# sidfeels/cosmos-predict2.5

Hardware: AMD Instinct MI355X
Metric: frames/sec, Predict2.5-2B Image2World 720p×121f, 35 UniPC steps, CP=1/8 (higher is better)
Workload: dtype bf16

## Files before the change

cosmos-predict2.5_amd/cosmos_predict2/_native.py:

```python

from __future__ import annotations

import ctypes
import os
from typing import Optional, Tuple

import torch

_DEFAULT_LIB_PATH = os.path.join(os.path.dirname(os.path.abspath(__file__)), "_lib", "libcp25.so")
_LIB_PATH = _DEFAULT_LIB_PATH
_lib: Optional[ctypes.CDLL] = None

c_int64_p = ctypes.POINTER(ctypes.c_int64)


class UniPCParams(ctypes.Structure):

    _fields_ = [
        ("sigma", ctypes.c_float),
        ("use_corr", ctypes.c_int),
        ("order_c", ctypes.c_int),
        ("c_a", ctypes.c_float),
        ("c_b", ctypes.c_float),
        ("c_c", ctypes.c_float),
# ... 21 lines not shown


DT_BF16, DT_F32, DT_F8E4M3, DT_U8 = 1, 2, 3, 4
_DTYPES = {torch.bfloat16: DT_BF16, torch.float32: DT_F32, torch.float8_e4m3fn: DT_F8E4M3, torch.uint8: DT_U8}

_P = ctypes.c_void_p
_I64 = ctypes.c_int64
_I = ctypes.c_int
_F = ctypes.c_float
_D = ctypes.c_double
_T =ctypes.POINTER(CP25Tensor)

SIGNATURES = {
    "cp25_attn_fwd": [_P, _P, _P, _P, _I, _I, _I, _I, _I, c_int64_p, c_int64_p, c_int64_p, c_int64_p, _F, _P],
    "cp25_attn_fwd_split": [_P, _P, _P, _P, _I, _I, _I, _I, _I, c_int64_p, c_int64_p, c_int64_p, c_int64_p, _F, _I,
                            _P, ctypes.c_size_t, _P],
    "cp25_attn_fwd_bounded": [_P, _P, _P, _P, _I, _I, _I, _I, _I, c_int64_p, c_int64_p, c_int64_p, c_int64_p, _F, _F,
                              _F, _I, _P, ctypes.c_size_t, _P],
    "cp25_attn_fwd_prescaled_kslots": [_P, _P, _P, _P, _I, _I, _I, _I, _I, c_int64_p, c_int64_p, c_int64_p, c_int64_p,
                                       _F, _F, _P, _I, _I, _P, ctypes.c_size_t, _P],
    "cp25_attn_fwd_prescaled": [_P, _P, _P, _P, _I, _I, _I, _I, _I, c_int64_p, c_int64_p, c_int64_p, c_int64_p, _F,
                                _F, _I, _P, ctypes.c_size_t, _P],
    "cp25_attn_fwd_prescaled_fp8qk": [_P, _P, _P, _P, _I, _I, _I, _I, _I, c_int64_p, c_int64_p, c_int64_p, c_int64_p, _F,
                                _F, _I, _P, ctypes.c_size_t, _P],
    "cp25_cast_fp8_e4m3": [_P, _I64, _P, _I64, _I64, _I64, _F, _P],
    "cp25_attn_fwd_prescaled_fp8": [_P, _P, _P, _P, _P, _I, _I, _I, _I, _I, c_int64_p, c_int64_p, c_int64_p, _F, _F, _I,
                                    _P, ctypes.c_size_t, _P],
    "cp25_v_fp8t_bytes": [_I, _I, _I],
    "cp25_cast_v_fp8t": [_P, c_int64_p, _I, _I, _I, _I, _P, _P, _P],
    "cp25_attn_fwd_prescaled_qnorm": [_P, _P, _P, _P, _I, _I, _I, _I, _I, c_int64_p, c_int64_p, c_int64_p, c_int64_p, _F,
                                      _F, _P, _I, _P, _P, _P, _F, _F, _I, _P, ctypes.c_size_t, _P],
    "cp25_attn_workspace_bytes": [_I, _I, _I, _I],
    "cp25_attn_tail_workspace_bytes": [_I, _I, _I, _I],
    "cp25_attn_kernel": [_I, _F, _F, _F, _I, _I],
    "cp25_attn_plan": [_I, _I, _I, _I, _I],
    "cp25_attn_na3d": [_P, _P, _P, _P, _I, _I, _I, _I, _I, _I, c_int64_p, c_int64_p, c_int64_p, c_int64_p, _P, _P, _I, _I,
                       ctypes.POINTER(ctypes.c_int), ctypes.POINTER(ctypes.c_int), _F, _I, _P],
    "cp25_ln_mod": [_P, _I64, _I64, _P, _P, _P, _P, _I64, _I64, _P, _P, _I64, _I, _I, _I64, _I64, _F, _P],
    "cp25_ln_mod_fp8": [_P, _I64, _I64, _P, _P, _P, _P, _I64, _I64, _P, _P, _P, _I64, _I, _I, _I64, _I64, _F, _P],
    "cp25_ln_mod_cam": [_P, _I64, _I64, _P, _P, _P, _P, _I64, _I64, _P, _I64, _I64, _P, _P, _I64, _I, _I, _I64, _I64, _F,
                        _P],
    "cp25_ln_mod_cam_fp8": [_P, _I64, _I64, _P, _P, _P, _P, _I64, _I64, _P, _I64, _I64, _P, _P, _P, _I64, _I, _I, _I64,
                            _I64, _F, _P],
    "cp25_plucker_tokens": [_P, _P, _P, _I, _I, _I, _P],
    "cp25_final_ln_mod": [_P, _P, _P, _I64, _I64, _P, _P, _I64, _I64, _P, _I64, _I, _I, _I64, _I64, _F, _P],
    "cp25_layer_norm": [_P, _I64, _P, _P, _P, _I64, _I64, _I, _F, _P],
    "cp25_head_rmsnorm_rope": [_P, _I64, _I64, _I, _I, _I, _P, _P, _P, _P, _I64, _F, _P],
    "cp25_head_rmsnorm_rope_scaled": [_P, _I64, _I64, _I, _I, _I, _P, _P, _P, _P, _I64, _F, _F, _P],
    "cp25_head_rmsnorm_rope_nmax": [_P, _I64, _I64, _I, _I, _I, _P, _P, _P, _P, _I64, _F, _F, _P, _P],
    "cp25_copy_rows": [_P, _I64, _P, _I64, _I64, _I64, _P],
    "cp25_gelu": [_P, _I64, _P],
    "cp25_gemm_epi": [_P, _I64, _P, _I64, _P, _I64, _I, _I, _I, _I, _P],
    "cp25_gemm_f32": [_P, _I64, _I64, _P, _I64, _I64, _P, _I64, _I64, _P, _I64, _I64, _I, _I, _I, _I, _I, _P, _I64,
                      _P],
    "cp25_gemm_f32_workspace_floats": [_I, _I, _I, _I],
    "cp25_gemm_hnorm": [_P, _I64, _P, _I64, _P, _I64, _I, _I, _I, _P, _F, _F, _P],
    "cp25_gemm_qkv": [_P, _I64, _P, _I64, _P, _I64, _I, _I, _I, _I, _I, _P, _P, _P, _I, _F, _P],
    "cp25_gemm_res": [_P, _I64, _P, _I64, _P, _I64, _I, _I, _I, _P, _I64, _I64, _P, _I64, _I64, _I, _I64, _I64, _P],
    "cp25_gemm_fp8": [_P, _I64, _P, _P, _I64, _P, _P, _I64, _I, _I, _I, _P],
    "cp25_gemm_fp8_res": [_P, _I64, _P, _P, _I64, _P, _P, _I64, _I, _I, _I, _P, _I64, _I64, _P, _I64, _I64, _I, _I64,
                          _I64, _P],
    "cp25_quant_fp8_rows": [_P, _P, _P, _I64, _I64, _P],
    "cp25_gelu_quant_fp8": [_P, _P, _P, _I64, _I64, _P],
    "cp25_patchify": [_P, _P, _P, _P, _P, _I64, _I64, _I64, _P],
    "cp25_patchify_ld": [_P, _P, _P, _P, _P, _I64, _I64, _I64, _I64, _P],
    "cp25_cfg_velocity": [_P, _I, _P, _P, _P, _F, _I, _P, _I64, _I64, _I64, _P],
# ... 17 lines not shown
    "cp25_gemm_epi_t": [_T, _T, _T, _I, _P],
    "cp25_conv3d_t": [_T, _I, _T, _T, _T, _I, _I, _I, _I, _I, _I, _P],
    "cp25_resize_crop_u8": [_P, c_int64_p, _I, _I, _I, _I, _P, c_int64_p, _P, _P, _P, _I, _P, _P, _P, _I, _I, _I, _I,
                            _I, _I, _I, _P],
    "cp25_u8_to_clip": [_P, c_int64_p, _I, _I, _I, _I, _P, _P],
    "cp25_clip_to_u8": [_P, c_int64_p, _I, _I, _I, _I, _P, c_int64_p, _P],
    "cp25_lora_merge": [_P, _I64, _P, _P, _I64, _I64, _I, _F, _P],
}


def library_path() -> str:
    return _LIB_PATH


def load_library() -> ctypes.CDLL:
    global _lib
    if _lib is not None:
        return _lib
    if not os.path.exists(_LIB_PATH):
        raise RuntimeError(
            f"libcp25.so not found at {_LIB_PATH}: build it with `make -C cosmos-predict2.5_amd/csrc` "
            "(or __graft_entry__.build()). There is no non-native fallback."
        )
    lib = ctypes.CDLL(_LIB_PATH)
    lab = os.path.abspath(_LIB_PATH) != os.path.abspath(_DEFAULT_LIB_PATH)
    for name, argtypes in SIGNATURES.items():
        fn = getattr(lib, name, None)
        if fn is None:
            if argtypes is None or lab:
                continue
            raise RuntimeError(f"libcp25.so does not export {name}")
        if argtypes is not None:
            fn.argtypes = argtypes
        fn.restype = {"cp25_attn_workspace_bytes": ctypes.c_size_t, "cp25_attn_tail_workspace_bytes": ctypes.c_size_t, "cp25_v_fp8t_bytes": ctypes.c_int64,
                      "cp25_gemm_f32_workspace_floats": ctypes.c_int64,
                      "cp25_attn_kernel": ctypes.c_char_p,
                      "cp25_vae_attn_workspace_bytes": ctypes.c_int64}.get(name, ctypes.c_int)
    _lib = lib
    return lib


_ERRORS = {-22: "invalid shape/stride/pointer", -95: "unsupported dtype/size", -5: "kernel launch failed"}


def _check(name: str, rc: int) -> None:
    if rc != 0:
        msg = f"{name} failed with code {rc} ({_ERRORS.get(rc, 'unknown')})"
        if rc == -5:
            raise RuntimeError(msg)
        raise ValueError(msg)


def _ptr(t: Optional[torch.Tensor]) -> Optional[int]:
    if t is None:
        return None
    if not t.is_cuda:
        raise RuntimeError("cp25 kernels need device (HBM) tensors; got a CPU tensor")
    return t.data_ptr()


def _stream(device: torch.device) -> int:
    return torch.cuda.current_stream(device).cuda_stream


def tensor_desc(t: Optional[torch.Tensor]) -> Optional[CP25Tensor]:
    if t is None:
        return None
# ... 55 lines not shown


def attn_plan(B: int, H: int, Lq: int, Lk: int, D: int = 128) -> int:
    n = load_library().cp25_attn_plan(B, H, Lq, Lk, D)
    _check("cp25_attn_plan", min(n, 0))
    return n


def attn_fwd(q: torch.Tensor, k: torch.Tensor, v: torch.Tensor, out: Optional[torch.Tensor] = None,
             softmax_scale: Optional[float] = None, n_split: Optional[int] = None,
             norm_bounds: Optional[Tuple[float, float]] = None, prescaled: bool = False,
             fp8_qk: Optional[Tuple[torch.Tensor, torch.Tensor]] = None,
             fp8_v: Optional[Tuple[torch.Tensor, torch.Tensor]] = None,
             k_norm_slots: Optional[torch.Tensor] = None, q_norm: Optional[dict] = None) -> torch.Tensor:
    lib = load_library()
    if q.dtype != torch.bfloat16 or k.dtype != torch.bfloat16 or v.dtype != torch.bfloat16:
        raise ValueError("attn_fwd expects bf16 q/k/v (attention() recasts to bf16 first)")
    B, Lq, H, D = q.shape
    Bk, Lk, Hk, Dk = k.shape
    if (Bk, Hk, Dk) != (B, H, D) or tuple(v.shape) != tuple(k.shape):
        raise ValueError(f"shape mismatch q{tuple(q.shape)} k{tuple(k.shape)} v{tuple(v.shape)}")
    for t in (q, k, v):
        if t.stride(3) != 1:
            raise ValueError("head dim must be contiguous")
    if out is None:
        out = torch.empty((B, Lq, H, D), dtype=torch.bfloat16, device=q.device)
    scale = float(D) ** -0.5 if softmax_scale is None else float(softmax_scale)
    planned = n_split is None and not _ATTN_SPLIT
    if n_split is None:
        n_split = min(_ATTN_SPLIT, (Lk + 63) // 64) if _ATTN_SPLIT else attn_plan(B, H, Lq, Lk, D)
    ws_bytes = lib.cp25_attn_workspace_bytes(B, H, Lq, n_split)
    if planned and n_split == 1 and fp8_qk is None and k_norm_slots is None:
        ws_bytes = lib.cp25_attn_tail_workspace_bytes(B, H, Lq, Lk)
    ws = torch.empty(((ws_bytes + 15) // 16 * 4,), dtype=torch.float32, device=q.device) if ws_bytes else None
    qb, kb = (0.0, 0.0) if norm_bounds is None else (float(norm_bounds[0]), float(norm_bounds[1]))
    if not (qb >= 0.0 and kb >= 0.0):
        raise ValueError(f"norm_bounds must be >= 0, got {norm_bounds}")
    strides = [_i64x3((t.stride(0), t.stride(1), t.stride(2))) for t in (q, k, v, out)]
    if prescaled:
        if fp8_qk is not None:
            if q_norm is not None:
                raise ValueError("q_norm: the fp8 forms read e4m3 copies of the normalised q")
            if qb * kb > 60.0 or qb <= 0.0 or kb <= 0.0:
                raise ValueError(f"fp8 Q K^T needs norm bounds with product <= 60, got {norm_bounds}")
            q8, k8 = fp8_qk
            if q8.dtype != torch.uint8 or k8.dtype != torch.uint8 or q8.shape != q.shape or k8.shape != k.shape:
                raise ValueError("fp8_qk: uint8 (e4m3 bit pattern) views shaped like q and k expected")
            if q8.stride(3) != 1 or k8.stride(3) != 1:
                raise ValueError("fp8_qk: head dim must be contiguous")
            strides[0] = _i64x3((q8.stride(0), q8.stride(1), q8.stride(2)))
            strides[1] = _i64x3((k8.stride(0), k8.stride(1), k8.stride(2)))
            if fp8_v is not None:
                if 1.13 * qb * kb > 30.0:
                    raise ValueError(f"fp8 P.V needs 1.13 x the norm-bound product <= 30, got {norm_bounds}")
                v8t, amax = fp8_v
                if v8t.dtype != torch.uint8 or v8t.numel() != lib.cp25_v_fp8t_bytes(B, H, Lk) or \
                        amax.dtype != torch.float32 or amax.numel() < B * H:
                    raise ValueError("fp8_v: (v8t uint8 of cp25_v_fp8t_bytes, v_amax float32 [B*H]) expected")
                rc = lib.cp25_attn_fwd_prescaled_fp8(_ptr(q8), _ptr(k8), _ptr(v8t), _ptr(amax), _ptr(out), B, H, Lq, Lk,
                                                     D, strides[0], strides[1], strides[3], qb, kb, int(n_split),
                                                     _ptr(ws), ws_bytes, _stream(q.device))
                _check("cp25_attn_fwd_prescaled_fp8", rc)
                return out
            rc = lib.cp25_attn_fwd_prescaled_fp8qk(_ptr(q8), _ptr(k8), _ptr(v), _ptr(out), B, H, Lq, Lk, D, *strides,
                                                   qb, kb, int(n_split), _ptr(ws), ws_bytes, _stream(q.device))
            _check("cp25_attn_fwd_prescaled_fp8qk", rc)
# ... 803 lines not shown
```

cosmos-predict2.5_amd/csrc/attn_common.h:

```cpp
#pragma once
#include "cp25_common.h"

#include <algorithm>
#include <type_traits>

namespace cp25attn {

constexpr int kD = 128;
constexpr int kWaves = 8;
constexpr int kQRows = 32;
constexpr int kQBlk = kWaves * kQRows;
constexpr int kKBlk = 64;
constexpr int kThreads = kWaves * 64;
constexpr float kTop = 96.f;
constexpr float kMaxBound = 98.f;
constexpr float kPDrop = 60.f;
constexpr float kGateFixed = 110.f;
constexpr float kTopF8 = 60.f;
constexpr float kLazy = 24.f;

typedef __attribute__((address_space(3))) const char* lds_char_ptr;

typedef float f32x2 __attribute__((ext_vector_type(2)));
typedef __bf16 bf16x2v __attribute__((ext_vector_type(2)));
// ... 42 lines not shown
  x = fmaxf(__uint_as_float(r[0]), __uint_as_float(r[1]));
  auto s = __builtin_amdgcn_permlane32_swap(__float_as_uint(x), __float_as_uint(x), false, false);
  return fmaxf(__uint_as_float(s[0]), __uint_as_float(s[1]));
}

struct AttnArgs {
  const unsigned short* q; const unsigned short* k; const unsigned short* v; unsigned short* o;
  int64_t q_sb, q_sl, q_sh;
  int64_t k_sb, k_sl, k_sh;
  int64_t v_sb, v_sl, v_sh;
  int64_t o_sb, o_sl, o_sh;
  int B, H, Lq, Lk;
  int nqb;
  int nsplit;
  int tps;
  int ntk_v;
  const float* v_amax;
  float s_init;
  float* o_part;
  float* lse_part;
  float scale_log2;
  float kbound;
  const float* kslots;
  int n_kslots;
  const unsigned short* qn_w;
  const float* qn_cos;
  const float* qn_sin;
  float qn_eps, qn_scale;
  int qn_row0;
#ifdef CP25_ATTN_PROBE
  unsigned long long* probe;
  int probe_t0, probe_wg;
#endif
};

constexpr int kKStride16 = 288;
constexpr int kVStride16 = 288;
constexpr int kKBuf16 = kKBlk * kKStride16;
constexpr int kVBuf16 = kKBlk * kVStride16;
constexpr int kLds16 = 2 * kKBuf16 + 2 * kVBuf16;

typedef void (*AttnKernel)(AttnArgs);
AttnKernel wq_kernel(int rows, int mode, bool tail);
constexpr int kWqThreads = 256;

}
```

cosmos-predict2.5_amd/csrc/attn_fwd.hip:

```cpp
#include "attn_common.h"

namespace {
using namespace cp25attn;

constexpr int kAheadDefault = 2;

constexpr bool kQCopyStagger = true;
constexpr int kOStr = 264;
constexpr int kQSlot = kQRows * kOStr;
constexpr int kLdsP = kLds16 + kWaves * kQSlot;

template <int kKind, bool kPre, int kMode, bool kPersist = false, int kGate = 0, int kTail = 0>
__global__ void __launch_bounds__(kThreads, 2) attn_fwd_m16(AttnArgs a) {
  __shared__ __attribute__((aligned(16))) char smem[kPersist ? kLdsP : kLds16];
  constexpr int KB1 = kKBuf16, VB0 = 2 * kKBuf16;
  static_assert(kMode >= 0 && kMode <= 2 && (kMode != 1 || kPre), "kMode: 0 fixed, 1 zero shift, 2 online");
  static_assert(!kPersist || (kKind == 1 && kMode != 0), "persistent form: cross-attention, zero shift or online");
  constexpr bool online = kMode == 2;
  constexpr bool kInit = kPre && kMode != 1;
  constexpr int kAhead = !kPersist ? 3 : kAheadDefault;

  const int tile = xcd_remap(blockIdx.x, gridDim.x);
  int blk0 = 0, blk_end = 0;
  if constexpr (kPersist) {
// ... 9 lines not shown
  const int Lk = min(a.Lk - key0, a.tps * kKBlk);
  const int ntk = (Lk + kKBlk - 1) / kKBlk;

  const int tid = threadIdx.x;
  const int lane = tid & 63;
  const int wave = tid >> 6;
  const int c16 = lane & 15;
  const int g = lane >> 4;
  const bool group_b = __builtin_amdgcn_readfirstlane(tid) >= kThreads / 2;
  const int wave_u = __builtin_amdgcn_readfirstlane(tid >> 6);
#ifdef CP25_ATTN_PROBE
  __shared__ unsigned long long probe_lds[kWaves * 32 * 4];
  unsigned long long probe_clk[4] = {0, 0, 0, 0};
  unsigned probe_resc = 0;
  const bool probe_on = !kPersist && kTail == 0 && a.probe != nullptr && (int)blockIdx.x < a.probe_wg;
  int probe_t = -1;
  unsigned long long probe_b2 = 0;
#define ATTN_STAMP(T, K)                                                                                    \
  do {                                                                                                      \
    if (probe_on && (unsigned)((T) - a.probe_t0) < 32u) {                                                   \
      __builtin_amdgcn_sched_barrier(0);                                                                    \
      unsigned long long ts_;                                                                               \
      asm volatile("s_memtime %0\n\ts_waitcnt lgkmcnt(0)" : "=s"(ts_)::"memory");                          \
      probe_lds[(wave_u * 32 + (T) - a.probe_t0) * 4 + (K)] = ts_;                                         \
      __builtin_amdgcn_sched_barrier(0);                                                                    \
    }                                                                                                       \
  } while (0)
#else
#define ATTN_STAMP(T, K) \
  do {                   \
  } while (0)
#endif

  const unsigned short* qp = a.q + b * a.q_sb + h * a.q_sh;
  const unsigned short* kp = a.k + b * a.k_sb + h * a.k_sh + (int64_t)key0 * a.k_sl;
  const unsigned short* vp = a.v + b * a.v_sb + h * a.v_sh + (int64_t)key0 * a.v_sl;

  const int ntiles = kPersist ? (blk_end - blk0) * ntk : ntk;
  const int copy_tile = kPersist && ntk > 1 ? (kQCopyStagger ? (int)(blockIdx.x % (unsigned)(ntk - 1)) : 0) : 0;

  const int u = tid & (kThreads / 2 - 1);
  const int srow = u >> 4, sch = u & 15;
  const int64_t sl = group_b ? a.k_sl : a.v_sl;
  const char* sbase = group_b ? (const char*)kp : (const char*)vp;
  const int st_off = (int)(srow * sl * 2) + sch * 16, st_step = (int)(16 * sl * 2);
  u32x4 st[4];
  auto load_tile = [&](int t) __attribute__((always_inline)) {
    const char* base;
    int kt;
    if constexpr (kPersist) {
      const int tb = t / ntk;
      kt = t - tb * ntk;
      const int bh_t = (blk0 + tb) / a.nqb;
      const int b_t = bh_t / a.H, h_t = bh_t % a.H;
      base = group_b ? (const char*)(a.k + b_t * a.k_sb + h_t * a.k_sh) : (const char*)(a.v + b_t * a.v_sb + h_t * a.v_sh);
    } else {
      kt = t;
      base = sbase;
    }
    const int rows = (kPersist && t >= ntiles) ? 0 : min(Lk - kt * kKBlk, kKBlk);
    const int nbytes = rows > 0 ? (int)((rows - 1) * sl * 2) + 2 * kD : 0;
    const auto rsrc = __builtin_amdgcn_make_buffer_rsrc((void*)(base + (int64_t)kt * kKBlk * sl * 2), (short)0, nbytes,
                                                        0x00020000);
    int off = st_off;
    if constexpr (kPersist) {
      const int uf = ((wave_u & 3) << 6) + lane_fresh();
// ... 101 lines not shown
#pragma unroll
          for (int q = 0; q < 4; ++q)
            x[s][q] = hn2_norm(x[s][q], rstd2,
                               f32x2{static_cast<float>(wv[s][2 * q]), static_cast<float>(wv[s][2 * q + 1])});
        f32x2 y[4][4];
#pragma unroll
        for (int s = 0; s < 4; ++s)
#pragma unroll
          for (int q = 0; q < 4; ++q) y[s][q] = x[s][q];
        if (rope) {
#pragma unroll
          for (int s = 0; s < 4; ++s)
#pragma unroll
            for (int q = 0; q < 4; ++q) {
              const f32x4 cc = rc[qh][s & 1][q >> 1], sn = rsn[qh][s & 1][q >> 1];
              const int o = 2 * (q & 1);
              y[s][q] = hn2_rope(x[s][q], x[s ^ 2][q], s < 2 ? -1.f : 1.f, f32x2{cc[o], cc[o + 1]},
                                 f32x2{sn[o], sn[o + 1]});
            }
        }
#pragma unroll
        for (int s = 0; s < 4; ++s)
#pragma unroll
          for (int q = 0; q < 4; ++q) {
            const bf16x2v h = __builtin_convertvector(y[s][q] * scale2, bf16x2v);
            qf[qh][s][2 * q] = h.x;
            qf[qh][s][2 * q + 1] = h.y;
          }
      }
    }
  }

  float gate_kbound = a.kbound;
  if constexpr (kGate != 0) {
    static_assert(kPre && !kPersist && ((kGate == 1 && kMode == 0) || (kGate == 2 && kMode == 2)), "gated pair");
    __shared__ float gate_max[kWaves];
    float km = lane < a.n_kslots ? a.kslots[32 * lane] : 0.f;
    float qm = 0.f;
#pragma unroll
    for (int qh = 0; qh < 2; ++qh) {
      float qq = 0.f;
#pragma unroll
      for (int s = 0; s < 4; ++s)
#pragma unroll
        for (int e = 0; e < 8; ++e) {
          const float x = static_cast<float>(qf[qh][s][e]);
          qq = fmaf(x, x, qq);
        }
      qm = fmaxf(qm, sqrtf(group4_sum(qq)));
    }
#pragma unroll
    for (int m = 32; m >= 1; m >>= 1) {
      km = fmaxf(km, __shfl_xor(km, m));
      qm = fmaxf(qm, __shfl_xor(qm, m));
    }
    if (lane == 0) gate_max[wave] = qm;
    __syncthreads();
#pragma unroll
    for (int w = 0; w < kWaves; ++w) qm = fmaxf(qm, gate_max[w]);
    const bool fixed_ok = km > 0.f && qm * km * 1.001f <= kGateFixed;
    gate_kbound = km * 1.001f;
    if (fixed_ok != (kGate == 1)) {
      if constexpr (kDmaK) asm volatile("s_waitcnt vmcnt(0)" ::: "memory");
      return;
    }
  }

// ... 372 lines not shown
#endif
      mfma_phase(PAR, std::true_type{});
      if constexpr (kDmaK) asm volatile("s_waitcnt vmcnt(0)" ::: "memory");
      __syncthreads();
    };
    for (int t = 0; t + 1 < ntiles; t += 2) {
      step(B0{}, t);
      step(B1{}, t + 1);
    }
    if (ntiles & 1) step(B0{}, ntiles - 1);
  }

#ifdef CP25_ATTN_PROBE
  if (probe_on) {
    asm volatile("s_memtime %0\n\ts_memrealtime %1\n\ts_waitcnt lgkmcnt(0)" : "=s"(probe_clk[2]), "=s"(probe_clk[3])::"memory");
    for (int i = lane; i < 128; i += 64)
      a.probe[((size_t)blockIdx.x * kWaves + wave_u) * 128 + i] = probe_lds[wave_u * 128 + i];
    if (lane < 5)
      a.probe[(size_t)a.probe_wg * kWaves * 128 + ((size_t)blockIdx.x * kWaves + wave_u) * 8 + lane] =
          lane == 0 ? probe_clk[0] : lane == 1 ? probe_clk[1] : lane == 2 ? probe_clk[2] : lane == 3 ? probe_clk[3]
                                                                                                    : probe_resc;
  }
#undef ATTN_STAMP
#endif
  if constexpr (kPersist) {
    store_block(blk_end - 1);
    return;
  }
#pragma unroll
  for (int qh = 0; qh < 2; ++qh) {
    const float l_tot = lsum[qh][0];
    const float inv = 1.f / l_tot;
    if (q_row[qh] >= a.Lq) continue;
    if (a.nsplit > 1) {
      const int64_t row = ((int64_t)(split * a.B + b) * a.H + h) * a.Lq + q_row[qh];
      float* op = a.o_part + row * kD + 4 * g;
#pragma unroll
      for (int db = 0; db < 8; ++db) {
        f32x4 w;
#pragma unroll
        for (int e = 0; e < 4; ++e) w[e] = o[db][qh][e] * inv;
        *reinterpret_cast<f32x4*>(op + 16 * db) = w;
      }
      if (g == 0) a.lse_part[row] = m_run[qh] + __log2f(l_tot);
    } else if constexpr (kKind == 1) {
      store_rows16(a.o + b * a.o_sb + h * a.o_sh + (int64_t)q_row[qh] * a.o_sl, qh, inv, g);
    } else {
      unsigned short* op = a.o + b * a.o_sb + h * a.o_sh + (int64_t)q_row[qh] * a.o_sl + 4 * g;
#pragma unroll
      for (int db = 0; db < 8; ++db) {
        u16x4 w;
#pragma unroll
        for (int e = 0; e < 4; ++e) w[e] = f2bf(o[db][qh][e] * inv);
        *reinterpret_cast<u16x4*>(op + 16 * db) = w;
      }
    }
  }
}

constexpr int kVStride = 320;
constexpr int kVBuf = kKBlk * kVStride;
constexpr int kLdsF8 = 2 * kVBuf + 2 * kKBlk * 144;

template <int kKind, int kF8>
__global__ void __launch_bounds__(kThreads, 2) attn_fwd_f8(AttnArgs a) {
  __shared__ __attribute__((aligned(16))) char smem[kLdsF8];
// ... 398 lines not shown
  double best_cost = 1e300;
  for (int s = 1; s <= 8 && s <= ntiles; ++s) {
    const int64_t tps = cdiv(ntiles, s);
    if (cdiv(ntiles, tps) != s) continue;
    double cost = split_cost(nwg, ntiles, s, rows, cus);
    if (s == 1) {
      TailSeg seg[kMaxTailSegs];
      size_t need;
      double saved;
      if (plan_tail(B, H, Lq, Lk, qblk, seg, &need, &saved) > 0) cost -= saved;
    }
    if (cost < best_cost * 0.995) { best_cost = cost; best = s; }
  }
  return best;
}

int m16_mode(float q_norm_bound, float k_norm_bound, float scale_log2, bool prescaled, bool whole_ok = false) {
  const double bb = (double)q_norm_bound * k_norm_bound * (prescaled ? 1.0 : scale_log2);
  if (!(q_norm_bound > 0.f && k_norm_bound > 0.f)) return 2;
  if (whole_ok && bb <= kGateFixed) return 0;
  if (bb > kMaxBound) return 2;
  return prescaled && bb <= kTop ? 1 : 0;
}

bool m16_gated(float q_norm_bound, float k_norm_bound, bool long_keys) {
  return long_keys ? m16_mode(q_norm_bound, k_norm_bound, 1.f, true, true) == 2
                   : m16_mode(q_norm_bound, k_norm_bound, 1.f, true) != 1;
}

int g_xattn_form = 1;

int wq_default_rows(int Lk) { return Lk > 8192 ? 384 : 320; }
int g_self_form = 1;
int wide_rows(bool prescaled, int fp8, bool gated, int Lk, int mode) {
  if (g_self_form == 0 || !prescaled || fp8 != 0 || gated || Lk <= 4096 || mode == 2) return 0;
  const int rows = g_self_form == 1 ? wq_default_rows(Lk) : g_self_form;
  return wq_kernel(rows, mode, false) ? rows : 0;
}

bool use_xattn_persistent(bool short_keys, int n_split, int mode, int64_t ntiles) {
  return g_xattn_form == 1 && short_keys && n_split == 1 && mode != 0 && ntiles >= 2;
}

}

extern "C" int cp25_attn_self_select(int form) {
  if (form != 0 && form != 1 && !wq_kernel(form, 0, false)) return CP25_ERR_INVAL;
  const int prev = g_self_form;
  g_self_form = form;
  return prev;
}

extern "C" int cp25_attn_cross_select(int form) {
  if (form != 0 && form != 1) return CP25_ERR_INVAL;
  const int prev = g_xattn_form;
  g_xattn_form = form;
  return prev;
}

#ifdef CP25_ATTN_PROBE
static unsigned long long* g_probe = nullptr;
static int g_probe_t0 = 0, g_probe_wg = 0;
extern "C" void cp25_attn_probe_set(unsigned long long* probe, int t0, int n_wg) {
  g_probe = probe;
  g_probe_t0 = t0;
  g_probe_wg = n_wg;
}
#endif

static int attn_launch(const void* q, const void* k, const void* v, void* o, int B, int H, int Lq, int Lk, int D,
                       const int64_t* q_strides, const int64_t* k_strides, const int64_t* v_strides,
// ... 5 lines not shown
  if (D != kD) return CP25_ERR_DTYPE;
  if (fp8qk && !prescaled) return CP25_ERR_INVAL;
  if (fp8 == 2 && (!v_amax || ((uintptr_t)v_amax & 3))) return CP25_ERR_INVAL;
  if (fp8qk && !(q_norm_bound > 0.f && k_norm_bound > 0.f && (double)q_norm_bound * k_norm_bound <= (double)kTopF8))
    return CP25_ERR_INVAL;
  if (fp8 == 2 && 1.13 * (double)q_norm_bound * k_norm_bound > 30.0) return CP25_ERR_INVAL;
  if (B <= 0 || H <= 0 || Lq <= 0 || Lk <= 0) return CP25_ERR_INVAL;
  if (!q || !k || !v || !o) return CP25_ERR_INVAL;
  if (!(softmax_scale > 0.f) || !(q_norm_bound >= 0.f) || !(k_norm_bound >= 0.f) || q_norm_bound > 1e18f ||
      k_norm_bound > 1e18f)
    return CP25_ERR_INVAL;
  const int64_t* ss[4] = {q_strides, k_strides, v_strides, o_strides};
  for (int i = 0; i < 4; ++i)
    for (int j = 0; j < 3; ++j)
      if (!(fp8 == 2 && i == 2) && ss[i][j] % (fp8qk && i < 2 ? 16 : 8) != 0) return CP25_ERR_INVAL;
  if ((int64_t)kKBlk * k_strides[1] * (fp8qk ? 1 : 2) >= (1ll << 31) ||
      (fp8 != 2 && (int64_t)kKBlk * v_strides[1] * 2 >= (1ll << 31)))
    return CP25_ERR_INVAL;
  if (k_strides[1] <= 0 || (fp8 != 2 && v_strides[1] <= 0)) return CP25_ERR_INVAL;
  if (((uintptr_t)q | (uintptr_t)k | (uintptr_t)v | (uintptr_t)o) & 15) return CP25_ERR_INVAL;
  const int64_t ntiles = cdiv(Lk, kKBlk);
  if (n_split < 1 || n_split > ntiles) return CP25_ERR_INVAL;
  const int64_t tps = cdiv(ntiles, n_split);
  if (cdiv(ntiles, tps) != n_split) return CP25_ERR_INVAL;
  const int64_t rows = (int64_t)B * H * Lq;
  if (n_split > 1) {
    if (!workspace || ((uintptr_t)workspace & 15) || ws_bytes < cp25_attn_workspace_bytes(B, H, Lq, n_split))
      return CP25_ERR_INVAL;
  }
  const bool xk = Lk <= 4096;
  const float sl2 = prescaled ? 1.f : softmax_scale * 1.4426950408889634f;
  const int mode = m16_mode(q_norm_bound, k_norm_bound, sl2, prescaled, !xk);
  const bool gated = prescaled && kslots && m16_gated(q_norm_bound, k_norm_bound, !xk);
  const int wq_rows = wide_rows(prescaled, fp8, gated, Lk, mode);
  const int qblk = wq_rows ? wq_rows : kQBlk;
  TailSeg tail[kMaxTailSegs];
  int n_tail = 0;
  if (n_split == 1 && fp8 == 0 && !kslots && workspace && !((uintptr_t)workspace & 15)) {
    size_t need = 0;
    n_tail = plan_tail(B, H, Lq, Lk, qblk, tail, &need, nullptr);
    if (ws_bytes < need) n_tail = 0;
  }
  AttnArgs a;
  a.q = (const unsigned short*)q; a.k = (const unsigned short*)k; a.v = (const unsigned short*)v;
  a.o = (unsigned short*)o;
  a.q_sb = q_strides[0]; a.q_sl = q_strides[1]; a.q_sh = q_strides[2];
  a.k_sb = k_strides[0]; a.k_sl = k_strides[1]; a.k_sh = k_strides[2];
  a.v_sb = v_strides[0]; a.v_sl = v_strides[1]; a.v_sh = v_strides[2];
  a.o_sb = o_strides[0]; a.o_sl = o_strides[1]; a.o_sh = o_strides[2];
  a.B = B; a.H = H; a.Lq = Lq; a.Lk = Lk;
  a.nqb = (int)cdiv(Lq, qblk);
  a.nsplit = n_split;
  a.tps = (int)tps;
  a.ntk_v = (int)ntiles;
  a.v_amax = v_amax;
  a.s_init = fp8 == 2 ? -std::max(0.f, 1.13f * q_norm_bound * k_norm_bound - 15.f) : 0.f;
  a.o_part = n_split > 1 ? (float*)workspace : nullptr;
  a.lse_part = n_split > 1 ? (float*)workspace + (size_t)n_split * rows * kD : nullptr;
  a.scale_log2 = sl2;
  a.kbound = q_norm_bound > 0.f ? k_norm_bound : 0.f;
  a.kslots = kslots;
  a.n_kslots = n_kslots;
  a.qn_w = qn ? qn->qn_w : nullptr;
  a.qn_cos = qn ? qn->qn_cos : nullptr;
  a.qn_sin = qn ? qn->qn_sin : nullptr;
  a.qn_eps = qn ? qn->qn_eps : 0.f;
  a.qn_scale = qn ? qn->qn_scale : 1.f;
  a.qn_row0 = 0;
#ifdef CP25_ATTN_PROBE
  a.probe = g_probe;
  a.probe_t0 = g_probe_t0;
  a.probe_wg = g_probe_wg;
#endif
  const int64_t nwg = (int64_t)a.nqb * B * H * n_split;
  if (nwg > 0x7fffffff) return CP25_ERR_INVAL;
  if (fp8 == 2) {
    hipLaunchKernelGGL((xk ? attn_fwd_f8<1, 3> : attn_fwd_f8<0, 3>), dim3((unsigned)nwg), dim3(kThreads), 0, stream, a);
  } else if (fp8qk) {
    hipLaunchKernelGGL((xk ? attn_fwd_f8<1, 1> : attn_fwd_f8<0, 1>), dim3((unsigned)nwg), dim3(kThreads), 0, stream, a);
  } else {
    void (*kern)(AttnArgs) = nullptr;
    void (*kern_tail)(AttnArgs) = nullptr;
    int64_t grid = nwg;
    int threads = kThreads;
    if (gated) {
      hipLaunchKernelGGL((xk ? attn_fwd_m16<1, true, 0, false, 1> : attn_fwd_m16<0, true, 0, false, 1>),
                         dim3((unsigned)nwg), dim3(kThreads), 0, stream, a);
      CP25_LAUNCH_CHECK();
      kern = xk ? attn_fwd_m16<1, true, 2, false, 2> : attn_fwd_m16<0, true, 2, false, 2>;
    } else if (!qn && use_xattn_persistent(xk, n_split, mode, ntiles)) {
      grid = std::min<int64_t>(nwg, num_cus());
      if (prescaled) kern = mode == 2 ? attn_fwd_m16<1, true, 2, true> : attn_fwd_m16<1, true, 1, true>;
      else kern = attn_fwd_m16<1, false, 2, true>;
    } else {
#define M16(P, M) kern = xk ? attn_fwd_m16<1, P, M> : attn_fwd_m16<0, P, M>; \
                  kern_tail = attn_fwd_m16<0, P, M, false, 0, 1>
      if (wq_rows) {
        kern = wq_kernel(wq_rows, mode, false);
        kern_tail = wq_kernel(wq_rows, mode, true);
        threads = kWqThreads;
      } else if (prescaled) {
        if (mode == 2) { M16(true, 2); } else if (mode == 1) { M16(true, 1); } else { M16(true, 0); }
      } else {
        if (mode == 2) { M16(false, 2); } else { M16(false, 0); }
      }
#undef M16
      if (n_tail) grid = nwg - nwg % num_cus();
    }
    hipLaunchKernelGGL(kern, dim3((unsigned)grid), dim3(threads), 0, stream, a);
    CP25_LAUNCH_CHECK();
    for (int i = grid < nwg ? 0 : n_tail; i < n_tail; ++i) {
      const TailSeg& g = tail[i];
      const int b = g.bh / H, h = g.bh % H;
      const int64_t row0 = (int64_t)g.qb_lo * qblk;
      AttnArgs t = a;
      t.q = a.q + b * a.q_sb + h * a.q_sh + row0 * a.q_sl;
      t.k = a.k + b * a.k_sb + h * a.k_sh;
      t.v = a.v + b * a.v_sb + h * a.v_sh;
// ... 27 lines not shown
                                             int Lq, int Lk, int D, const int64_t* q_strides,
                                             const int64_t* k_strides, const int64_t* v_strides,
                                             const int64_t* o_strides, float q_norm_bound, float k_norm_bound,
                                             int n_split, void* workspace, size_t ws_bytes, hipStream_t stream) {
  return attn_launch(q8, k8, v, o, B, H, Lq, Lk, D, q_strides, k_strides, v_strides, o_strides, 0.6931471805599453f,
                     q_norm_bound, k_norm_bound, n_split, workspace, ws_bytes, stream, true, 1);
}

extern "C" int cp25_attn_fwd_prescaled_fp8(const void* q8, const void* k8, const void* v8t, const float* v_amax,
                                           void* o, int B, int H, int Lq, int Lk, int D, const int64_t* q_strides,
                                           const int64_t* k_strides, const int64_t* o_strides, float q_norm_bound,
                                           float k_norm_bound, int n_split, void* workspace, size_t ws_bytes,
                                           hipStream_t stream) {
  const int64_t none[3] = {0, 0, 0};
  return attn_launch(q8, k8, v8t, o, B, H, Lq, Lk, D, q_strides, k_strides, none, o_strides, 0.6931471805599453f,
                     q_norm_bound, k_norm_bound, n_split, workspace, ws_bytes, stream, true, 2, v_amax);
}

extern "C" size_t cp25_attn_workspace_bytes(int B, int H, int Lq, int n_split) {
  if (n_split <= 1 || B <= 0 || H <= 0 || Lq <= 0) return 0;
  return (size_t)n_split * B * H * Lq * (kD + 1) * sizeof(float);
}

extern "C" size_t cp25_attn_tail_workspace_bytes(int B, int H, int Lq, int Lk) {
  if (B <= 0 || H <= 0 || Lq <= 0 || Lk <= 0) return 0;
  TailSeg seg[kMaxTailSegs];
  size_t need = 0, best = 0;
  const int wide = g_self_form == 0 ? 0 : (g_self_form == 1 ? wq_default_rows(Lk) : g_self_form);
  for (int qblk : {kQBlk, Lk > 4096 ? wide : 0})
    if (qblk > 0 && plan_tail(B, H, Lq, Lk, qblk, seg, &need, nullptr) > 0) best = std::max(best, need);
  return best;
}

extern "C" int cp25_attn_plan(int B, int H, int Lq, int Lk, int D) {
  if (D != kD) return CP25_ERR_DTYPE;
  if (B <= 0 || H <= 0 || Lq <= 0 || Lk <= 0) return CP25_ERR_INVAL;
  return plan_split(B, H, Lq, Lk, kQBlk);
}

extern "C" int cp25_attn_fwd(const void* q, const void* k, const void* v, void* o, int B, int H, int Lq,
                             int Lk, int D, const int64_t* q_strides, const int64_t* k_strides,
                             const int64_t* v_strides, const int64_t* o_strides, float softmax_scale,
                             hipStream_t stream) {
  return attn_launch(q, k, v, o, B, H, Lq, Lk, D, q_strides, k_strides, v_strides, o_strides, softmax_scale, 0.f,
                     0.f, 1, nullptr, 0, stream);
}

extern "C" int cp25_attn_fwd_split(const void* q, const void* k, const void* v, void* o, int B, int H, int Lq,
                                   int Lk, int D, const int64_t* q_strides, const int64_t* k_strides,
                                   const int64_t* v_strides, const int64_t* o_strides, float softmax_scale,
                                   int n_split, void* workspace, size_t ws_bytes, hipStream_t stream) {
  return attn_launch(q, k, v, o, B, H, Lq, Lk, D, q_strides, k_strides, v_strides, o_strides, softmax_scale, 0.f,
                     0.f, n_split, workspace, ws_bytes, stream);
}

extern "C" int cp25_attn_fwd_bounded(const void* q, const void* k, const void* v, void* o, int B, int H, int Lq,
                                     int Lk, int D, const int64_t* q_strides, const int64_t* k_strides,
                                     const int64_t* v_strides, const int64_t* o_strides, float softmax_scale,
                                     float q_norm_bound, float k_norm_bound, int n_split, void* workspace,
                                     size_t ws_bytes, hipStream_t stream) {
  return attn_launch(q, k, v, o, B, H, Lq, Lk, D, q_strides, k_strides, v_strides, o_strides, softmax_scale,
                     q_norm_bound, k_norm_bound, n_split, workspace, ws_bytes, stream);
}

extern "C" int cp25_attn_fwd_prescaled(const void* q, const void* k, const void* v, void* o, int B, int H, int Lq,
                                       int Lk, int D, const int64_t* q_strides, const int64_t* k_strides,
// ... 10 lines not shown
                                              float k_norm_bound, const float* k_norm_slots, int n_slots, int n_split,
                                              void* workspace, size_t ws_bytes, hipStream_t stream) {
  if (!k_norm_slots || n_slots < 1 || n_slots > 64 || ((uintptr_t)k_norm_slots & 3)) return CP25_ERR_INVAL;
  return attn_launch(q, k, v, o, B, H, Lq, Lk, D, q_strides, k_strides, v_strides, o_strides, 0.6931471805599453f,
                     q_norm_bound, k_norm_bound, n_split, workspace, ws_bytes, stream, true, 0, nullptr, k_norm_slots,
                     n_slots);
}

extern "C" int cp25_attn_fwd_prescaled_qnorm(const void* q, const void* k, const void* v, void* o, int B, int H, int Lq,
                                             int Lk, int D, const int64_t* q_strides, const int64_t* k_strides,
                                             const int64_t* v_strides, const int64_t* o_strides, float q_norm_bound,
                                             float k_norm_bound, const float* k_norm_slots, int n_slots,
                                             const void* q_norm_weight, const float* cos_tab, const float* sin_tab,
                                             float eps, float q_scale, int n_split, void* workspace, size_t ws_bytes,
                                             hipStream_t stream) {
  if (k_norm_slots && (n_slots < 1 || n_slots > 64 || ((uintptr_t)k_norm_slots & 3))) return CP25_ERR_INVAL;
  if (!q_norm_weight || ((uintptr_t)q_norm_weight & 15) || (!cos_tab) != (!sin_tab) || !(eps >= 0.f) ||
      !(q_scale > 0.f))
    return CP25_ERR_INVAL;
  if ((((uintptr_t)cos_tab) | ((uintptr_t)sin_tab)) & 15) return CP25_ERR_INVAL;
  AttnArgs qn{};
  qn.qn_w = (const unsigned short*)q_norm_weight;
  qn.qn_cos = cos_tab;
  qn.qn_sin = sin_tab;
  qn.qn_eps = eps;
  qn.qn_scale = q_scale;
  return attn_launch(q, k, v, o, B, H, Lq, Lk, D, q_strides, k_strides, v_strides, o_strides, 0.6931471805599453f,
                     q_norm_bound, k_norm_bound, n_split, workspace, ws_bytes, stream, true, 0, nullptr, k_norm_slots,
                     k_norm_slots ? n_slots : 0, &qn);
}

extern "C" const char* cp25_attn_kernel(int Lk, float softmax_scale, float q_norm_bound, float k_norm_bound,
                                        int prescaled, int fp8) {
  if (prescaled == 2 && m16_gated(q_norm_bound, k_norm_bound, Lk > 4096))
    return Lk <= 4096 ? "attn_fwd_m16<cross, prescaled, gated fixed shift | online max>"
                      : "attn_fwd_m16<self, prescaled, gated fixed shift | online max>";
  if (fp8 == 2) return Lk <= 4096 ? "attn_fwd_f8<cross, fp8 Q K^T + fp8 P.V>" : "attn_fwd_f8<self, fp8 Q K^T + fp8 P.V>";
  if (fp8 == 1) return Lk <= 4096 ? "attn_fwd_f8<cross, fp8 Q K^T>" : "attn_fwd_f8<self, fp8 Q K^T>";
  if (Lk <= 4096) {
    const float sl = prescaled ? 1.f : softmax_scale * 1.4426950408889634f;
    const int mode = m16_mode(q_norm_bound, k_norm_bound, sl, prescaled != 0);
    if (use_xattn_persistent(true, 1, mode, cdiv(Lk, kKBlk)))
      return mode == 1 ? "attn_fwd_m16<cross, prescaled, zero shift, persistent>"
                       : (prescaled ? "attn_fwd_m16<cross, prescaled, online max, persistent>"
                                    : "attn_fwd_m16<cross, online max, persistent>");
  }
  if (Lk > 4096 && prescaled) {
    const int mode = m16_mode(q_norm_bound, k_norm_bound, 1.f, true, true);
    const int rows = wide_rows(true, fp8, false, Lk, mode);
    static const char* wq[2][2] = {
        {"attn_fwd_wq<self, prescaled, 320 rows, fixed shift>", "attn_fwd_wq<self, prescaled, 320 rows, zero shift>"},
        {"attn_fwd_wq<self, prescaled, 384 rows, fixed shift>", "attn_fwd_wq<self, prescaled, 384 rows, zero shift>"}};
    if (rows) return wq[rows == 384][mode];
  }
  static const char* names[2][2][3] = {
      {{"attn_fwd_m16<self, fixed shift>", "?", "attn_fwd_m16<self, online max>"},
       {"attn_fwd_m16<self, prescaled, fixed shift>", "attn_fwd_m16<self, prescaled, zero shift>",
        "attn_fwd_m16<self, prescaled, online max>"}},
      {{"attn_fwd_m16<cross, fixed shift>", "?", "attn_fwd_m16<cross, online max>"},
       {"attn_fwd_m16<cross, prescaled, fixed shift>", "attn_fwd_m16<cross, prescaled, zero shift>",
        "attn_fwd_m16<cross, prescaled, online max>"}}};
  const float sl = prescaled ? 1.f : softmax_scale * 1.4426950408889634f;
  return names[Lk <= 4096][prescaled != 0][m16_mode(q_norm_bound, k_norm_bound, sl, prescaled != 0, Lk > 4096)];
}
```

cosmos-predict2.5_amd/csrc/attn_wide.hip:

```cpp
#include "attn_common.h"

namespace cp25attn {
namespace {

constexpr int kAheadWq = 2;
constexpr int kRingWq = kAheadWq + 1;
static_assert(kWqThreads == 4 * 64, "one wave per SIMD");

constexpr int wq_stage(int nq) { return 17 * nq; }
constexpr int wq_frag(int nq, int m) { return m < nq ? -1 : (m - nq) / nq; }
constexpr int wq_qb(int nq, int m) { return m < nq ? m : (m - nq) % nq; }
constexpr bool wq_read_gap(int nq, int m) { return m >= nq && (m - nq) % nq == 0; }
constexpr int wq_sm_op(int nq, int m) {
  if (wq_read_gap(nq, m)) return -1;
  int idx = 0;
  for (int x = 0; x < m; ++x) idx += !wq_read_gap(nq, x);
  return idx < 12 * nq ? idx : -1;
}
constexpr int wq_sm_count(int nq) {
  int n = 0;
  for (int m = 0; m < wq_stage(nq); ++m) n += wq_sm_op(nq, m) >= 0;
  return n;
}
static_assert(wq_sm_count(5) == 60 && wq_sm_count(6) == 72, "every softmax instruction has a gap");
// ... 142 lines not shown
#pragma unroll
          for (int q = 0; q < 4; ++q) {
            const f32x4 cc = rc[s & 1][q >> 1], sn = rsn[s & 1][q >> 1];
            const int o = 2 * (q & 1);
            y[s][q] = hn2_rope(x[s][q], x[s ^ 2][q], s < 2 ? -1.f : 1.f, f32x2{cc[o], cc[o + 1]},
                               f32x2{sn[o], sn[o + 1]});
          }
      }
#pragma unroll
      for (int s = 0; s < 4; ++s)
#pragma unroll
        for (int q = 0; q < 4; ++q) {
          const bf16x2v hh = __builtin_convertvector(y[s][q] * scale2, bf16x2v);
          qa[qb][s][2 * q] = hh.x;
          qa[qb][s][2 * q + 1] = hh.y;
        }
    }
  }

  float m_run[kNQ];
#pragma unroll
  for (int qb = 0; qb < kNQ; ++qb) m_run[qb] = 0.f;
  if constexpr (kMode == 0) {
#pragma unroll
    for (int qb = 0; qb < kNQ; ++qb) {
      float qq = 0.f;
#pragma unroll
      for (int s = 0; s < 4; ++s)
#pragma unroll
        for (int e = 0; e < 8; ++e) {
          const float x = static_cast<float>(qa[qb][s][e]);
          qq = fmaf(x, x, qq);
        }
      const float b_row = sqrtf(group4_sum(qq)) * a.kbound;
      m_run[qb] = floorf(fminf(b_row + kPDrop, 126.f - b_row));
    }
  }
  f32x4 minit[kNQ];
#pragma unroll
  for (int qb = 0; qb < kNQ; ++qb) {
    minit[qb] = f32x4{-m_run[qb], -m_run[qb], -m_run[qb], -m_run[qb]};
    asm volatile("" : "+v"(minit[qb]));
  }

  f32x4 oacc[8][kNQ], lacc[kNQ];
#pragma unroll
  for (int db = 0; db < 8; ++db)
#pragma unroll
    for (int qb = 0; qb < kNQ; ++qb) {
      oacc[db][qb] = f32x4{0.f, 0.f, 0.f, 0.f};
      asm volatile("s_nop 2" : "+a"(oacc[db][qb]));
    }
#pragma unroll
  for (int qb = 0; qb < kNQ; ++qb) {
    lacc[qb] = f32x4{0.f, 0.f, 0.f, 0.f};
    asm volatile("s_nop 2" : "+a"(lacc[qb]));
  }
  static_for<kNQ>([&](auto QC) __attribute__((always_inline)) {
    constexpr int qb = decltype(QC)::value;
    (void)qa;
#pragma unroll
    for (int s = 0; s < 4; ++s) {
      if constexpr (qb < kQA) asm volatile("s_nop 2" : "+a"(qa[qb][s]));
      else asm volatile("s_nop 2" : "+v"(qa[qb][s]));
    }
  });
  typedef short s16x8v __attribute__((ext_vector_type(8)));
// ... 235 lines not shown
```

include/cp25.h:

```cpp
#ifndef CP25_H
#define CP25_H

#include <stdint.h>
#include <hip/hip_runtime_api.h>

#ifdef __cplusplus
extern "C" {
#endif

#define CP25_MAX_DIMS 6
#define CP25_DT_BF16 1
#define CP25_DT_F32 2
#define CP25_DT_F8E4M3 3
#define CP25_DT_U8 4
typedef struct cp25_tensor {
  void* data;
  int32_t dtype;
  int32_t ndim;
  int64_t shape[CP25_MAX_DIMS];
  int64_t strides[CP25_MAX_DIMS];
} cp25_tensor;

int cp25_attn_fwd_t(const cp25_tensor* q, const cp25_tensor* k, const cp25_tensor* v, const cp25_tensor* o,
                    float softmax_scale, void* workspace, size_t ws_bytes, hipStream_t stream);
// ... 31 lines not shown
                                   size_t ws_bytes, hipStream_t stream);

int cp25_attn_fwd_prescaled_qnorm(const void* q, const void* k, const void* v, void* o, int B, int H, int Lq, int Lk,
                                  int D, const int64_t* q_strides, const int64_t* k_strides, const int64_t* v_strides,
                                  const int64_t* o_strides, float q_norm_bound, float k_norm_bound,
                                  const float* k_norm_slots, int n_slots, const void* q_norm_weight,
                                  const float* cos_tab, const float* sin_tab, float eps, float q_scale, int n_split,
                                  void* workspace, size_t ws_bytes, hipStream_t stream);

int cp25_cast_fp8_e4m3(const void* src, int64_t src_stride, void* dst, int64_t dst_stride, int64_t n_rows,
                       int64_t width, float scale, hipStream_t stream);

int cp25_attn_fwd_prescaled_fp8qk(const void* q8, const void* k8, const void* v, void* o, int B, int H, int Lq, int Lk,
                                  int D, const int64_t* q_strides, const int64_t* k_strides, const int64_t* v_strides,
                                  const int64_t* o_strides, float q_norm_bound, float k_norm_bound, int n_split,
                                  void* workspace, size_t ws_bytes, hipStream_t stream);

int64_t cp25_v_fp8t_bytes(int B, int H, int L);
int cp25_cast_v_fp8t(const void* v, const int64_t* v_strides, int B, int H, int L, int D, void* v8t, float* v_amax,
                     hipStream_t stream);

int cp25_attn_fwd_prescaled_fp8(const void* q8, const void* k8, const void* v8t, const float* v_amax, void* o, int B,
                                int H, int Lq, int Lk, int D, const int64_t* q_strides, const int64_t* k_strides,
                                const int64_t* o_strides, float q_norm_bound, float k_norm_bound, int n_split,
                                void* workspace, size_t ws_bytes, hipStream_t stream);

const char* cp25_attn_kernel(int Lk, float softmax_scale, float q_norm_bound, float k_norm_bound, int prescaled,
                             int fp8);

size_t cp25_attn_workspace_bytes(int B, int H, int Lq, int n_split);

size_t cp25_attn_tail_workspace_bytes(int B, int H, int Lq, int Lk);

int cp25_attn_plan(int B, int H, int Lq, int Lk, int D);

int cp25_attn_cross_select(int form);

int cp25_attn_self_select(int form);

int cp25_attn_na3d(const void* q, const void* k, const void* v, void* o, int B, int H, int T, int Hg, int Wg, int D,
                   const int64_t* q_strides, const int64_t* k_strides, const int64_t* v_strides,
                   const int64_t* o_strides, const int* q_tok, const int* box, int n_tiles, int tile_rows,
                   const int* window, const int* dilation, float softmax_scale, int prescaled, hipStream_t stream);

int cp25_ln_mod(const void* x, int64_t x_st, int64_t x_sb, const void* y, const void* gate, const void* shift,
                const void* scale, int64_t mod_sb, int64_t mod_st, void* x_out, void* h_out, int64_t n_tok, int B,
                int D, int64_t tok0, int64_t hw, float eps, hipStream_t stream);

int cp25_ln_mod_fp8(const void* x, int64_t x_st, int64_t x_sb, const void* y, const void* gate, const void* shift,
                    const void* scale, int64_t mod_sb, int64_t mod_st, void* x_out, void* h8_out, float* h_scale,
                    int64_t n_tok, int B, int D, int64_t tok0, int64_t hw, float eps, hipStream_t stream);

int cp25_ln_mod_cam(const void* x, int64_t x_st, int64_t x_sb, const void* y, const void* gate, const void* shift,
                    const void* scale, int64_t mod_sb, int64_t mod_st, const void* cam, int64_t cam_st, int64_t cam_sb,
                    void* x_out, void* h_out, int64_t n_tok, int B, int D, int64_t tok0, int64_t hw, float eps,
                    hipStream_t stream);
int cp25_ln_mod_cam_fp8(const void* x, int64_t x_st, int64_t x_sb, const void* y, const void* gate, const void* shift,
                        const void* scale, int64_t mod_sb, int64_t mod_st, const void* cam, int64_t cam_st,
                        int64_t cam_sb, void* x_out, void* h8_out, float* h_scale, int64_t n_tok, int B, int D,
                        int64_t tok0, int64_t hw, float eps, hipStream_t stream);

int cp25_final_ln_mod(const void* x, const void* y, const void* gate, int64_t gmod_sb, int64_t gmod_st,
                      const float* shift, const float* scale, int64_t mod_sb, int64_t mod_st, float* out,
                      int64_t n_tok, int B, int D, int64_t tok0, int64_t hw, float eps, hipStream_t stream);

int cp25_layer_norm(const void* x, int64_t x_stride, const void* weight, const void* bias, void* y, int64_t y_stride,
// ... 136 lines not shown
```

Baseline: 0.8298.

## Route gated self-attention through the wide-query kernel with per-tile fallback flags

Gated self-attention (per-key-slot norm bounds) previously could not use the wide-row attention kernel. The wide kernel now computes the gate itself, using the max query norm per tile times the max key-slot norm. When the fixed-shift softmax is safe it runs the fast path; otherwise it writes a fallback flag to a new workspace and exits. A second online-max launch then reprocesses only the flagged rows, skipping blocks whose flags are clear. This adds a workspace query in the Python binding and risks extra launch overhead when many tiles fail the gate.

New measurement: 0.8296, median of 2. No clear change (-0.0%).

```diff
diff --git a/cosmos-predict2.5_amd/cosmos_predict2/_native.py b/cosmos-predict2.5_amd/cosmos_predict2/_native.py
--- a/cosmos-predict2.5_amd/cosmos_predict2/_native.py
+++ b/cosmos-predict2.5_amd/cosmos_predict2/_native.py
@@ -77,6 +77,7 @@
                                       _F, _P, _I, _P, _P, _P, _F, _F, _I, _P, ctypes.c_size_t, _P],
     "cp25_attn_workspace_bytes": [_I, _I, _I, _I],
     "cp25_attn_tail_workspace_bytes": [_I, _I, _I, _I],
+    "cp25_attn_gate_workspace_bytes": [_I, _I, _I, _I],
     "cp25_attn_kernel": [_I, _F, _F, _F, _I, _I],
     "cp25_attn_plan": [_I, _I, _I, _I, _I],
     "cp25_attn_na3d": [_P, _P, _P, _P, _I, _I, _I, _I, _I, _I, c_int64_p, c_int64_p, c_int64_p, c_int64_p, _P, _P, _I, _I,
@@ -160,7 +161,8 @@
             raise RuntimeError(f"libcp25.so does not export {name}")
         if argtypes is not None:
             fn.argtypes = argtypes
-        fn.restype = {"cp25_attn_workspace_bytes": ctypes.c_size_t, "cp25_attn_tail_workspace_bytes": ctypes.c_size_t, "cp25_v_fp8t_bytes": ctypes.c_int64,
+        fn.restype = {"cp25_attn_workspace_bytes": ctypes.c_size_t, "cp25_attn_tail_workspace_bytes": ctypes.c_size_t,
+                      "cp25_attn_gate_workspace_bytes": ctypes.c_size_t, "cp25_v_fp8t_bytes": ctypes.c_int64,
                       "cp25_gemm_f32_workspace_floats": ctypes.c_int64,
                       "cp25_attn_kernel": ctypes.c_char_p,
                       "cp25_vae_attn_workspace_bytes": ctypes.c_int64}.get(name, ctypes.c_int)
@@ -282,6 +284,8 @@
     ws_bytes = lib.cp25_attn_workspace_bytes(B, H, Lq, n_split)
     if planned and n_split == 1 and fp8_qk is None and k_norm_slots is None:
         ws_bytes = lib.cp25_attn_tail_workspace_bytes(B, H, Lq, Lk)
+    if n_split == 1 and prescaled and fp8_qk is None and k_norm_slots is not None:
+        ws_bytes = lib.cp25_attn_gate_workspace_bytes(B, H, Lq, Lk)
     ws = torch.empty(((ws_bytes + 15) // 16 * 4,), dtype=torch.float32, device=q.device) if ws_bytes else None
     qb, kb = (0.0, 0.0) if norm_bounds is None else (float(norm_bounds[0]), float(norm_bounds[1]))
     if not (qb >= 0.0 and kb >= 0.0):
diff --git a/cosmos-predict2.5_amd/csrc/attn_common.h b/cosmos-predict2.5_amd/csrc/attn_common.h
--- a/cosmos-predict2.5_amd/csrc/attn_common.h
+++ b/cosmos-predict2.5_amd/csrc/attn_common.h
@@ -98,6 +98,8 @@
   unsigned long long* probe;
   int probe_t0, probe_wg;
 #endif
+  unsigned* gate_flags;
+  int gate_rows, gate_nqb;
 };
 
 constexpr int kKStride16 = 288;
diff --git a/cosmos-predict2.5_amd/csrc/attn_fwd.hip b/cosmos-predict2.5_amd/csrc/attn_fwd.hip
--- a/cosmos-predict2.5_amd/csrc/attn_fwd.hip
+++ b/cosmos-predict2.5_amd/csrc/attn_fwd.hip
@@ -65,6 +65,19 @@
   } while (0)
 #endif
 
+  unsigned gate_f0 = 0, gate_f1 = 0;
+  int gate_row1 = 0;
+  if constexpr (kGate == 3) {
+    static_assert(kKind == 0 && kPre && !kPersist && kMode == 2, "the wide gated pair's second launch: online max");
+    const int r0 = qb * kQBlk, r1 = min(r0 + kQBlk, a.Lq) - 1;
+    const int w0 = r0 / a.gate_rows, w1 = r1 / a.gate_rows;
+    const unsigned* fl = a.gate_flags + (int64_t)bh * a.gate_nqb;
+    gate_f0 = fl[w0];
+    gate_f1 = fl[w1];
+    gate_row1 = (w0 + 1) * a.gate_rows;
+    if ((gate_f0 | gate_f1) == 0) return;
+  }
+
   const unsigned short* qp = a.q + b * a.q_sb + h * a.q_sh;
   const unsigned short* kp = a.k + b * a.k_sb + h * a.k_sh + (int64_t)key0 * a.k_sl;
   const unsigned short* vp = a.v + b * a.v_sb + h * a.v_sh + (int64_t)key0 * a.v_sl;
@@ -232,7 +245,7 @@
   }
 
   float gate_kbound = a.kbound;
-  if constexpr (kGate != 0) {
+  if constexpr (kGate == 1 || kGate == 2) {
     static_assert(kPre && !kPersist && ((kGate == 1 && kMode == 0) || (kGate == 2 && kMode == 2)), "gated pair");
     __shared__ float gate_max[kWaves];
     float km = lane < a.n_kslots ? a.kslots[32 * lane] : 0.f;
@@ -671,6 +684,9 @@
     const float l_tot = lsum[qh][0];
     const float inv = 1.f / l_tot;
     if (q_row[qh] >= a.Lq) continue;
+    if constexpr (kGate == 3) {
+      if ((q_row[qh] < gate_row1 ? gate_f0 : gate_f1) == 0) continue;
+    }
     if (a.nsplit > 1) {
       const int64_t row = ((int64_t)(split * a.B + b) * a.H + h) * a.Lq + q_row[qh];
       float* op = a.o_part + row * kD + 4 * g;
@@ -1135,11 +1151,16 @@
 
 int wq_default_rows(int Lk) { return Lk > 8192 ? 384 : 320; }
 int g_self_form = 1;
-int wide_rows(bool prescaled, int fp8, bool gated, int Lk, int mode) {
-  if (g_self_form == 0 || !prescaled || fp8 != 0 || gated || Lk <= 4096 || mode == 2) return 0;
-  const int rows = g_self_form == 1 ? wq_default_rows(Lk) : g_self_form;
-  return wq_kernel(rows, mode, false) ? rows : 0;
-}
+int wide_width(int Lk) {
+  if (g_self_form == 0 || Lk <= 4096) return 0;
+  return g_self_form == 1 ? wq_default_rows(Lk) : g_self_form;
+}
+int wide_rows(bool prescaled, int fp8, bool gated, int Lk, int mode, bool gate_ws = false) {
+  if (!prescaled || fp8 != 0 || (gated ? !gate_ws : mode == 2)) return 0;
+  const int rows = wide_width(Lk);
+  return rows && wq_kernel(rows, gated ? 0 : mode, false) ? rows : 0;
+}
+size_t gate_ws_bytes(int B, int H, int Lq, int rows) { return sizeof(unsigned) * (size_t)B * H * cdiv(Lq, rows); }
 
 bool use_xattn_persistent(bool short_keys, int n_split, int mode, int64_t ntiles) {
   return g_xattn_form == 1 && short_keys && n_split == 1 && mode != 0 && ntiles >= 2;
@@ -1211,7 +1232,10 @@
   const float sl2 = prescaled ? 1.f : softmax_scale * 1.4426950408889634f;
   const int mode = m16_mode(q_norm_bound, k_norm_bound, sl2, prescaled, !xk);
   const bool gated = prescaled && kslots && m16_gated(q_norm_bound, k_norm_bound, !xk);
-  const int wq_rows = wide_rows(prescaled, fp8, gated, Lk, mode);
+  const int gw = wide_width(Lk);
+  const bool gate_ws = gated && gw && n_split == 1 && workspace && !((uintptr_t)workspace & 3) &&
+                       ws_bytes >= gate_ws_bytes(B, H, Lq, gw);
+  const int wq_rows = wide_rows(prescaled, fp8, gated, Lk, mode, gate_ws);
   const int qblk = wq_rows ? wq_rows : kQBlk;
   TailSeg tail[kMaxTailSegs];
   int n_tail = 0;
@@ -1246,6 +1270,9 @@
   a.qn_eps = qn ? qn->qn_eps : 0.f;
   a.qn_scale = qn ? qn->qn_scale : 1.f;
   a.qn_row0 = 0;
+  a.gate_flags = nullptr;
+  a.gate_rows = 0;
+  a.gate_nqb = 0;
 #ifdef CP25_ATTN_PROBE
   a.probe = g_probe;
   a.probe_t0 = g_probe_t0;
@@ -1262,7 +1289,17 @@
     void (*kern_tail)(AttnArgs) = nullptr;
     int64_t grid = nwg;
     int threads = kThreads;
-    if (gated) {
+    if (gated && wq_rows) {
+      grid = cdiv(Lq, kQBlk) * B * H;
+      if (grid > 0x7fffffff) return CP25_ERR_INVAL;
+      a.gate_flags = (unsigned*)workspace;
+      a.gate_rows = wq_rows;
+      a.gate_nqb = a.nqb;
+      hipLaunchKernelGGL(wq_kernel(wq_rows, 0, false), dim3((unsigned)nwg), dim3(kWqThreads), 0, stream, a);
+      CP25_LAUNCH_CHECK();
+      a.nqb = (int)cdiv(Lq, kQBlk);
+      kern = attn_fwd_m16<0, true, 2, false, 3>;
+    } else if (gated) {
       hipLaunchKernelGGL((xk ? attn_fwd_m16<1, true, 0, false, 1> : attn_fwd_m16<0, true, 0, false, 1>),
                          dim3((unsigned)nwg), dim3(kThreads), 0, stream, a);
       CP25_LAUNCH_CHECK();
@@ -1356,6 +1393,12 @@
   return best;
 }
 
+extern "C" size_t cp25_attn_gate_workspace_bytes(int B, int H, int Lq, int Lk) {
+  if (B <= 0 || H <= 0 || Lq <= 0 || Lk <= 0) return 0;
+  const int rows = wide_width(Lk);
+  return rows && wq_kernel(rows, 0, false) ? gate_ws_bytes(B, H, Lq, rows) : 0;
+}
+
 extern "C" int cp25_attn_plan(int B, int H, int Lq, int Lk, int D) {
   if (D != kD) return CP25_ERR_DTYPE;
   if (B <= 0 || H <= 0 || Lq <= 0 || Lk <= 0) return CP25_ERR_INVAL;
@@ -1432,9 +1475,14 @@
 
 extern "C" const char* cp25_attn_kernel(int Lk, float softmax_scale, float q_norm_bound, float k_norm_bound,
                                         int prescaled, int fp8) {
-  if (prescaled == 2 && m16_gated(q_norm_bound, k_norm_bound, Lk > 4096))
+  if (prescaled == 2 && m16_gated(q_norm_bound, k_norm_bound, Lk > 4096)) {
+    const int rows = wide_rows(true, fp8, true, Lk, 2, true);
+    if (rows)
+      return rows == 384 ? "attn_fwd_m16<self, prescaled, gated attn_fwd_wq<384 rows, fixed shift> | online max>"
+                         : "attn_fwd_m16<self, prescaled, gated attn_fwd_wq<320 rows, fixed shift> | online max>";
     return Lk <= 4096 ? "attn_fwd_m16<cross, prescaled, gated fixed shift | online max>"
                       : "attn_fwd_m16<self, prescaled, gated fixed shift | online max>";
+  }
   if (fp8 == 2) return Lk <= 4096 ? "attn_fwd_f8<cross, fp8 Q K^T + fp8 P.V>" : "attn_fwd_f8<self, fp8 Q K^T + fp8 P.V>";
   if (fp8 == 1) return Lk <= 4096 ? "attn_fwd_f8<cross, fp8 Q K^T>" : "attn_fwd_f8<self, fp8 Q K^T>";
   if (Lk <= 4096) {
diff --git a/cosmos-predict2.5_amd/csrc/attn_wide.hip b/cosmos-predict2.5_amd/csrc/attn_wide.hip
--- a/cosmos-predict2.5_amd/csrc/attn_wide.hip
+++ b/cosmos-predict2.5_amd/csrc/attn_wide.hip
@@ -198,7 +198,35 @@
           const float x = static_cast<float>(qa[qb][s][e]);
           qq = fmaf(x, x, qq);
         }
-      const float b_row = sqrtf(group4_sum(qq)) * a.kbound;
+      m_run[qb] = sqrtf(group4_sum(qq));
+    }
+    float kb = a.kbound;
+    if (a.kslots != nullptr) {
+      __shared__ float gate_max[4];
+      float km = lane < a.n_kslots ? a.kslots[32 * lane] : 0.f;
+      float qm = 0.f;
+#pragma unroll
+      for (int qb = 0; qb < kNQ; ++qb) qm = fmaxf(qm, m_run[qb]);
+#pragma unroll
+      for (int m = 32; m >= 1; m >>= 1) {
+        km = fmaxf(km, __shfl_xor(km, m));
+        qm = fmaxf(qm, __shfl_xor(qm, m));
+      }
+      if (lane == 0) gate_max[wave] = qm;
+      __syncthreads();
+#pragma unroll
+      for (int w = 0; w < 4; ++w) qm = fmaxf(qm, gate_max[w]);
+      const bool fixed_ok = km > 0.f && qm * km * 1.001f <= kGateFixed;
+      if (tid == 0) a.gate_flags[tile] = fixed_ok ? 0u : 1u;
+      if (!fixed_ok) {
+        asm volatile("s_waitcnt vmcnt(0)" ::: "memory");
+        return;
+      }
+      kb = km * 1.001f;
+    }
+#pragma unroll
+    for (int qb = 0; qb < kNQ; ++qb) {
+      const float b_row = m_run[qb] * kb;
       m_run[qb] = floorf(fminf(b_row + kPDrop, 126.f - b_row));
     }
   }
diff --git a/include/cp25.h b/include/cp25.h
--- a/include/cp25.h
+++ b/include/cp25.h
@@ -87,6 +87,8 @@
 
 size_t cp25_attn_tail_workspace_bytes(int B, int H, int Lq, int Lk);
 
+size_t cp25_attn_gate_workspace_bytes(int B, int H, int Lq, int Lk);
+
 int cp25_attn_plan(int B, int H, int Lq, int Lk, int D);
 
 int cp25_attn_cross_select(int form);
```
